# tensorflow/compression

Hardware: AMD Instinct MI355X
Metric: Mpixels/s encode+decode round-trip (bit-exact) (higher is better)
Workload: dtype int32

## Files before the change

compression_amd/csrc/range_pipe.h:

```cpp
#pragma once

#ifndef TFC_PIPE_TIMING
#define TFC_PIPE_TIMING 0
#endif

namespace tfc {

constexpr int kPipeTile = 256;
constexpr int kPipeEscMax = 32;
constexpr unsigned int kPipeBlock = 16;
constexpr unsigned int kPipeNoCall = 0x0001FFFFu;
constexpr unsigned int kPipeAggregate = 1u << 30;
constexpr unsigned int kPipePrefix = 2u << 30;
constexpr unsigned int kPipeRowsMask = (1u << 30) - 1u;

struct PipeEncArgs {
  const uint16_t* fast16;
  const int2* rows_fast;
  int ntab;
  int tab_entries;
  unsigned int* calls;
  unsigned int* status;
  unsigned int* done;
  unsigned int* fallback;
// ... 591 lines not shown
    const unsigned int dslot = b % L::kDigSlots;
    dstage = area + L::kDig + dslot * L::kDigSlot + L::kDigStride * lane;
    ds_off = area_off + L::kDig + dslot * L::kDigSlot + L::kDigStride * lane;
    n = 0u;
    block(wa);
    if (lane == 0u) sync[L::kConsumed] = b + 1u;
    if (!last) {
      seq = ((seq_early & ~(L::kLast | L::kBail)) == b + 2u || (seq_early & L::kBail)) ? seq_early : wait_words(b + 1u);
      if (seq & L::kBail) { bail = true; break; }
      read_words(wa, (b + 1u) % L::kSlots, 0u);
    }
    block(wb);
    reinterpret_cast<uint2*>(area + L::kRec)[dslot * 64u + lane] = make_uint2(wpos, n);
    overflow |= (n != 0u && wpos + ((n + 15u) & ~15u) > pa.cap) ? 1u : 0u;
    wpos += n;
    asm volatile("s_waitcnt lgkmcnt(0)" ::: "memory");
    if (lane == 0u) sync[L::kDigPub] = b + 1u;
    if (__any(too_long)) {
      bail = true;
      if (lane == 0u) atomicOr(&pa.fallback[job], 1u);
      break;
    }
    if (last) break;
  }
  asm volatile("s_waitcnt lgkmcnt(0)" ::: "memory");
  if (lane == 0u) sync[L::kExit] = 1u;
  if (gi == 0u && lane == 0u) {
    g_pipe_clock[0] = clock64() - clk0;
    g_pipe_clock[1] = wall_clock64() - wall0;
    g_pipe_clock[4] = waited_words;
    g_pipe_clock[6] = waited_digits;
#if TFC_PIPE_TIMING
    g_enc_clock[0] = t_blocks; g_enc_clock[1] = n_blocks; g_enc_clock[2] = n_redone; g_enc_clock[3] = t_redo;
#endif
  }
  if (bail) return;
  if (live) {
    pa.stage_state[static_cast<size_t>(gi) * 64 + lane] = make_uint4(base, s1, (hd & 0xFFFFu) | (had << 31), rn);
    pa.stage_out[static_cast<size_t>(gi) * 64 + lane] = make_uint2(wpos, overflow);
  }
}

__global__ void __launch_bounds__(64) enc_chain_direct_kernel(const PipeChainJobs jobs, const PipeEncArgs pa) {
  constexpr unsigned int kRows = PipeEncChainLds::kRows;
  constexpr unsigned int kDigits = 2 * kRows;
  constexpr int kStride = lane_stride(kDigits + 8);
  __shared__ __attribute__((aligned(16))) unsigned char stage[64 * kStride];
  const unsigned int gi = blockIdx.x;
  const unsigned int job = gi / static_cast<unsigned int>(pa.groups_per_job);
  const unsigned int gidx = gi % static_cast<unsigned int>(pa.groups_per_job);
  if (__hip_atomic_load(&pa.fallback[job], __ATOMIC_RELAXED, __HIP_MEMORY_SCOPE_AGENT) != 0u) return;
  const PipeChainJob& J = jobs.job[job];
  const unsigned int lane = threadIdx.x;
  const int64_t s = static_cast<int64_t>(gidx) * 64 + lane;
  const bool live = s < jobs.streams;

  uint4 st = live ? J.state[s] : make_uint4(0u, 0xFFFFFFFFu, 0u, 0u);
  unsigned int base = st.x, s1 = st.y, hd = st.z & 0xFFFFu, had = st.z >> 31, rn = st.w;
  lanes_pin(base, s1, hd, rn);

  const unsigned int ds_off = static_cast<unsigned int>(reinterpret_cast<size_t>(
                                  (__attribute__((address_space(3))) unsigned char*)stage)) + kStride * lane;
  unsigned char* const dstage = stage + kStride * lane;
  unsigned char* const out = J.chunk + (live ? s : 0) * static_cast<int64_t>(pa.cap);
  unsigned int wpos = 0u, n = 0u, overflow = 0u;

  auto put = [&](unsigned int d, bool on) {
    *reinterpret_cast<unsigned short*>(dstage + n) = __builtin_bswap16(static_cast<unsigned short>(d));
    n += on ? 2u : 0u;
  };
  auto flush = [&]() {
#pragma unroll
    for (unsigned int c = 0; c < kDigits / 16u; ++c) {
      if (16u * c < n) {
        uint2 v[2];
        v[0] = reinterpret_cast<const uint2*>(dstage)[2 * c];
        v[1] = reinterpret_cast<const uint2*>(dstage)[2 * c + 1];
        if (wpos + 16u * c + 16u <= pa.cap) lanes_gstore16(out + wpos + 16u * c, v[0], v[1]);
        else overflow = 1u;
      }
    }
    wpos += n;
    n = 0u;
  };
  auto put_run = [&](unsigned int fill, unsigned int bytes) {
    flush();
    for (unsigned int k = 0; k < bytes; k += 2u) {
      const unsigned short be = static_cast<unsigned short>(fill);
      if (wpos + 2u <= pa.cap) lanes_gstore_elem(reinterpret_cast<unsigned short*>(out + wpos), be);
      else overflow = 1u;
      wpos += 2u;
    }
  };
  auto call = [&](unsigned int lo, unsigned int hi, bool act) __attribute__((always_inline)) {
    const unsigned int a = scale16(s1, lo);
    const unsigned int b = scale16(s1, hi) - 1u;
    const unsigned int bs = base + a;
    const unsigned int t1 = b - a;
    const bool carry = act && bs < a;
    const bool ren = act && (t1 >> 16) == 0u;
    const unsigned int e = bs >> 16;
    const bool solid = ren && e != 0xFFFFu;
    const bool ffff = ren && e == 0xFFFFu;
    const bool held = had != 0u;
    const unsigned int X = (hd + (carry ? 1u : 0u)) & 0xFFFFu;
    const bool emit = held && (solid || (carry && (!ffff || rn != 0u)));
    put(X, emit);
    const unsigned int run_out = !held ? 0u : solid ? rn : (carry && rn != 0u) ? (ffff ? rn - 1u : rn) : 0u;
    if (__any(run_out != 0u)) {
      if (run_out != 0u) put_run(carry ? 0u : 0xFFFFu, 2u * run_out);
    }
    if (solid) {
      hd = e; had = 1u; rn = 0u;
    } else if (ffff) {
      if (!held) { hd = 0xFFFFu; had = 1u; rn = 0u; }
      else if (!carry) { rn += 1u; }
      else if (rn == 0u) { hd = X; rn = 1u; }
      else { hd = 0u; rn = 1u; }
    } else if (carry && held) {
      had = 0u; rn = 0u;
    }
    base = act ? (ren ? bs << 16 : bs) : base;
    s1 = act ? (ren ? (t1 << 16) | 0xFFFFu : t1) : s1;
  };

  const unsigned int nt = static_cast<unsigned int>(pa.nt);
  const unsigned int* const status = pa.status + static_cast<size_t>(gi) * nt * 64 + lane;
  const unsigned int* const done = pa.done + static_cast<size_t>(gi) * nt;
  unsigned int avail = 0u;
  unsigned int tn = 0u;
  bool bail = false;
  auto ensure = [&](unsigned int need) {
    while (tn < nt && __any(live && avail < need)) {
      const unsigned int* const flag = done + tn;
      long long t0 = 0;
      bool timing = false;
      while (__hip_atomic_load(flag, __ATOMIC_RELAXED, __HIP_MEMORY_SCOPE_AGENT) == 0u) {
        const long long now = static_cast<long long>(wall_clock64());
        if (!timing) { t0 = now; timing = true; }
        else if (now - t0 > pa.poll_ticks) { bail = true; return; }
        __builtin_amdgcn_s_sleep(8);
      }
      __builtin_amdgcn_fence(__ATOMIC_ACQUIRE, "agent");
      avail = __hip_atomic_load(status + static_cast<size_t>(tn) * 64, __ATOMIC_RELAXED, __HIP_MEMORY_SCOPE_AGENT) & kPipeRowsMask;
      ++tn;
      if (__hip_atomic_load(&pa.fallback[job], __ATOMIC_RELAXED, __HIP_MEMORY_SCOPE_AGENT) != 0u) { bail = true; return; }
    }
  };

  const unsigned char* const mine = reinterpret_cast<const unsigned char*>(pa.calls + static_cast<size_t>(gi) * 64 * pa.rows) + 128u * lane;
  unsigned int w[kRows] = {}, wn[kRows] = {};
  auto load_rows = [&](unsigned int b) {
    const unsigned char* p = mine + static_cast<size_t>(b) * (64u * kRows * 4u);
#pragma unroll
    for (unsigned int c = 0; c < kRows / 4u; ++c) {
      const uint4 v = lanes_gload16(p + 16u * c);
      wn[4 * c] = v.x; wn[4 * c + 1] = v.y; wn[4 * c + 2] = v.z; wn[4 * c + 3] = v.w;
    }
  };
  auto block = [&](unsigned int w0, unsigned int w1, unsigned int w2, unsigned int w3, unsigned int w4, unsigned int w5,
                   unsigned int w6, unsigned int w7, unsigned int w8, unsigned int w9, unsigned int w10, unsigned int w11,
                   unsigned int w12, unsigned int w13, unsigned int w14, unsigned int w15) __attribute__((always_inline)) {
    const unsigned int base0 = base, s10 = s1, hd0 = hd, had0 = had;
    unsigned int flag = rn, na = ds_off + n;
    asm volatile(
        "s_mov_b64 s[56:57], exec\n\t"
        "v_mov_b32 v101, 0\n\tv_mov_b32 v103, 0\n\t"
        TFC_PENC_STEP(W0) TFC_PENC_STEP(W1) TFC_PENC_STEP(W2) TFC_PENC_STEP(W3)
        TFC_PENC_STEP(W4) TFC_PENC_STEP(W5) TFC_PENC_STEP(W6) TFC_PENC_STEP(W7)
        TFC_PENC_STEP(W8) TFC_PENC_STEP(W9) TFC_PENC_STEP(W10) TFC_PENC_STEP(W11)
        TFC_PENC_STEP(W12) TFC_PENC_STEP(W13) TFC_PENC_STEP(W14) TFC_PENC_STEP(W15)
        "s_mov_b64 exec, s[56:57]\n\t"
        "s_waitcnt lgkmcnt(0)\n\t"
        : [BASE] "+v"(base), [S] "+v"(s1), [H] "+v"(hd), [HAD] "+v"(had), [NA] "+v"(na), [FLAG] "+v"(flag)
        : [NOCALL] "s"(kPipeNoCall), [K64K] "s"(0x10000u), [KFFFF] "s"(0xFFFFu), [PERM] "s"(0x0c0c0001u),
          [W0] "v"(w0), [W1] "v"(w1), [W2] "v"(w2), [W3] "v"(w3), [W4] "v"(w4), [W5] "v"(w5),
          [W6] "v"(w6), [W7] "v"(w7), [W8] "v"(w8), [W9] "v"(w9), [W10] "v"(w10), [W11] "v"(w11),
          [W12] "v"(w12), [W13] "v"(w13), [W14] "v"(w14), [W15] "v"(w15)
        : "vcc", "memory", "s52", "s53", "s56", "s57", "v100", "v101", "v102", "v103", "v104", "v105", "v106", "v107",
          "v108", "v109", "v110", "v111", "v112", "v113", "v114", "v115", "v117", "v118", "v119");
    if (__builtin_expect(!__any(flag != 0u), 1)) {
      n = na - ds_off;
    } else {
      base = base0; s1 = s10; hd = hd0; had = had0;
      const unsigned int ww[kPipeBlock] = {w0, w1, w2, w3, w4, w5, w6, w7, w8, w9, w10, w11, w12, w13, w14, w15};
#pragma nounroll
      for (unsigned int k = 0; k < kPipeBlock; ++k) {
        unsigned int word = ww[0];
#pragma unroll
        for (unsigned int q = 1; q < kPipeBlock; ++q) word = k == q ? ww[q] : word;
        const unsigned int hi = word >> 16;
        call(word & 0xFFFFu, hi == 0u ? 65536u : hi, word != kPipeNoCall);
      }
    }
  };

  ensure(kRows);
  if (!bail) load_rows(0u);
#pragma unroll
  for (unsigned int k = 0; k < kRows; ++k) asm volatile("" : "+v"(wn[k]));
  for (unsigned int b = 0; !bail && (tn < nt || __any(b * kRows < avail)); ++b) {
#pragma unroll
    for (unsigned int k = 0; k < kRows; ++k) w[k] = wn[k];
    ensure((b + 2u) * kRows);
    if (bail) break;
    load_rows(b + 1u);
    flush();
    if (__any(avail < (b + 1u) * kRows)) {
#pragma unroll
      for (unsigned int k = 0; k < kRows; ++k) w[k] = b * kRows + k < avail ? w[k] : kPipeNoCall;
    }
    block(w[0], w[1], w[2], w[3], w[4], w[5], w[6], w[7], w[8], w[9], w[10], w[11], w[12], w[13], w[14], w[15]);
    block(w[16], w[17], w[18], w[19], w[20], w[21], w[22], w[23], w[24], w[25], w[26], w[27], w[28], w[29], w[30], w[31]);
  }
  flush();
  if (bail) {
    if (lane == 0) atomicOr(&pa.fallback[job], 1u);
    return;
  }
  if (live) {
    pa.stage_state[static_cast<size_t>(gi) * 64 + lane] = make_uint4(base, s1, (hd & 0xFFFFu) | (had << 31), rn);
    pa.stage_out[static_cast<size_t>(gi) * 64 + lane] = make_uint2(wpos, overflow);
  }
}


__global__ void enc_gate_kernel(const unsigned int* started, unsigned int want, long long ticks) {
  const long long t0 = static_cast<long long>(wall_clock64());
  while (__hip_atomic_load(started, __ATOMIC_RELAXED, __HIP_MEMORY_SCOPE_AGENT) < want &&
         static_cast<long long>(wall_clock64()) - t0 < ticks)
    __builtin_amdgcn_s_sleep(8);
}

__global__ void __launch_bounds__(64) enc_commit_kernel(const PipeChainJobs jobs, const PipeEncArgs pa) {
  const unsigned int gi = blockIdx.x;
  const unsigned int job = gi / static_cast<unsigned int>(pa.groups_per_job);
  const unsigned int gidx = gi % static_cast<unsigned int>(pa.groups_per_job);
  if (pa.fallback[job] != 0u) return;
  const int64_t s = static_cast<int64_t>(gidx) * 64 + threadIdx.x;
  if (s >= jobs.streams) return;
  const PipeChainJob& J = jobs.job[job];
  J.state[s] = pa.stage_state[static_cast<size_t>(gi) * 64 + threadIdx.x];
  const uint2 o = pa.stage_out[static_cast<size_t>(gi) * 64 + threadIdx.x];
  J.chunk_len[s] = o.y ? 0u : o.x;
  if (o.y) atomicOr(J.overflow_flag, 1u);
}


constexpr unsigned int kPipeSkipRow = 0xFFFFu;
__device__ inline unsigned int pipe_raw_entry(unsigned int sym_or_bit, int M) { return (M != 0 ? 0x8000u : 0u) | sym_or_bit; }
__device__ inline int pipe_mode_step(int M, unsigned int bit) {
  if (M < 0) return bit ? -M : (M == -31 ? 32 : M - 1);
  return M - 1;
}

struct PipeDecArgs {
  unsigned short* raw;
  unsigned int* posrec;
  unsigned int* kend;
  uint4* state_out;
  const unsigned short* rowaddr;
  unsigned int* fallback;
  unsigned int* progress;
  unsigned int* tile_done;
  unsigned int* started;
  int rows;
  int groups_per_job;
  int groups;
  int concurrent;
  long long poll_ticks;
};
constexpr unsigned int kPipeFinal = 0x80000000u;
#ifndef TFC_PIPE_RELEASE
#define TFC_PIPE_RELEASE 64
#endif
constexpr unsigned int kPipeRelease = TFC_PIPE_RELEASE;
struct PipeDecJob { const uint8_t* blob; const long long* off; const uint4* state; };
struct PipeDecJobs {
  int64_t streams, elems;
  int blocks_per_job, n;
  PipeDecJob job[64];
};

struct PipeRowJobs {
  int64_t per_job;
  int ntab, n;
  struct { const int32_t* index; unsigned long long* first_error; } job[64];
};
__global__ void __launch_bounds__(256) dec_rows_kernel(const PipeRowJobs jobs, unsigned short* rowaddr) {
  const int k = blockIdx.y;
  const int32_t* index = jobs.job[k].index;
  unsigned short* out = rowaddr + static_cast<size_t>(k) * jobs.per_job;
  for (int64_t i = static_cast<int64_t>(blockIdx.x) * 1024 + threadIdx.x, e = min(jobs.per_job, (static_cast<int64_t>(blockIdx.x) + 1) * 1024);
       i < e; i += 256) {
    int t = tfc_gload(index + i);
    if (t < 0 || t >= jobs.ntab) {
      atomicMin(jobs.job[k].first_error, static_cast<unsigned long long>(i));
      t = 0;
    }
    out[i] = static_cast<unsigned short>(16 * t);
  }
}

struct PipeDecLds {
  static constexpr int kWords = 2 * kPipeBlock * 2 / 8 + 2;
  static constexpr int kStride = lane_stride(8 * kWords);
  static constexpr int kCodes = 0;
  static constexpr int kRows = kCodes + 64 * kStride;
  static constexpr int kBytes = kRows + 64 * kStride;
  static constexpr int kStage = kPipeBlock * 128;
};

#ifndef TFC_PDEC_ABL
#define TFC_PDEC_ABL 0
#endif
#if TFC_PDEC_ABL & 1
#define TFC_PDEC_STORE(KOFF)
#define TFC_PDEC_WAIT2 "s_waitcnt lgkmcnt(1)\n\t"
#else
#define TFC_PDEC_STORE(KOFF) "ds_write_b16 %[STG], v117 offset:" #KOFF "\n\t"
#define TFC_PDEC_WAIT2 "s_waitcnt lgkmcnt(2)\n\t"
#endif
#ifndef TFC_PDEC_PAD
#define TFC_PDEC_PAD 0
#endif
#define TFC_PDEC_PAD2 "v_mov_b32 v139, v139\n\tv_mov_b32 v139, v139\n\t"
#if TFC_PDEC_PAD == 1
#define TFC_PDEC_PAD_A TFC_PDEC_PAD2
#elif TFC_PDEC_PAD == 5
#define TFC_PDEC_PAD_A "s_waitcnt lgkmcnt(15)\n\ts_waitcnt lgkmcnt(15)\n\t"
#else
#define TFC_PDEC_PAD_A
#endif
#if TFC_PDEC_PAD == 2
#define TFC_PDEC_PAD_B TFC_PDEC_PAD2
#else
#define TFC_PDEC_PAD_B
#endif
#if TFC_PDEC_PAD == 3
#define TFC_PDEC_PAD_C TFC_PDEC_PAD2
#else
#define TFC_PDEC_PAD_C
#endif
#if TFC_PDEC_PAD == 4
#define TFC_PDEC_PAD_D TFC_PDEC_PAD2
#else
#define TFC_PDEC_PAD_D
#endif
#define TFC_PDEC_STEP(KOFF, MI, MO, AHEAD, NEXT, PWSTEP)                                    \
  "v_cvt_f32_u32 v111, %[S]\n\t"                                                          \
  "v_add_f32 v111, 1.0, v111\n\t"                                                         \
  "v_rcp_f32 v111, v111\n\t"                                                              \
  TFC_PDEC_PAD_A                                                                          \
  "v_cvt_f32_u32 v110, %[D]\n\t"                                                          \
  "v_fma_f32 v110, -v110, %[SCALE], -%[HSCALE]\n\t"                                       \
  "v_fma_f32 v110, v110, v111, -1.0\n\t"                                                  \
  "v_cvt_i32_f32 v110, v110\n\t"                                                          \
  "v_ashrrev_i32 v111, 6, v110\n\t"                                                       \
  "s_waitcnt lgkmcnt(0)\n\t"                                                              \
  "v_mad_i32_i24 v112, v111, -8, v106\n\t"                                                \
  "ds_read_b64 v[114:115], v112\n\t"                                                      \
  "v_mad_i32_i24 v113, v111, -2, v107\n\t"                                                \
  "ds_read_u16 v116, v113\n\t"                                                            \
  AHEAD                                                                                   \
  "v_cndmask_b32_e64 v133, 0, 2, s[56:57]\n\t"                                            \
  "v_add_u32 %[CP], %[CP], v133\n\t"                                                      \
  "ds_read_u16 v109, %[CP]\n\t"                                                           \
  "v_ashrrev_i32 v137, 31, " MI "\n\t"                                                    \
  "v_cmp_le_u32_sdwa vcc, v110, v105 src0_sel:WORD_0 src1_sel:WORD_1\n\t"                 \
  "v_cndmask_b32 v137, v136, v137, vcc\n\t"                                               \
  "v_xor_b32 " MO ", v135, v137\n\t"                                                      \
  "v_cmpx_le_u32 vcc, v130, v131\n\t"                                                     \
  TFC_PDEC_PAD_B                                                                          \
  "s_waitcnt lgkmcnt(1)\n\t"                                                              \
  "v_lshlrev_b64 v[118:119], v110, v[114:115]\n\t"                                        \
  "v_bcnt_u32_b32 v116, v118, v116\n\t"                                                   \
  "v_bcnt_u32_b32 v117, v119, v116\n\t"                                                   \
  "v_lshl_add_u32 v112, v117, 1, v104\n\t"                                                \
  "ds_read_u16 v122, v112 offset:2\n\t"                                                   \
  "ds_read_u16 v124, v112 offset:4\n\t"                                                   \
  TFC_PDEC_PAD_C                                                                          \
  TFC_PDEC_STORE(KOFF)                                                                    \
  "v_subrev_co_u32 v135, vcc, 1, " MO "\n\t"                                              \
  "v_cndmask_b32_e64 v136, 0, -1, vcc\n\t"                                                \
  "v_add_u32 v140, " #PWSTEP ", %[PW]\n\t"                                                \
  "v_cndmask_b32 %[PW], %[PW], v140, vcc\n\t"                                             \
  "v_cndmask_b32 v142, %[BINROW], " NEXT ", vcc\n\t"                                      \
  "ds_read_b128 v[104:107], v142\n\t"                                                     \
  TFC_PDEC_WAIT2                                                                          \
  TFC_PDEC_PAD_D                                                                          \
  "v_mad_u64_u32 v[126:127], s[52:53], v122, %[S], v[122:123]\n\t"                        \
  "v_mad_u64_u32 v[128:129], s[52:53], v124, %[S], v[124:125]\n\t"                        \
  "v_alignbit_b32 v126, v127, v126, 16\n\t"                                               \
  "v_alignbit_b32 v128, v129, v128, 16\n\t"                                               \
  "v_add_u32 v128, -1, v128\n\t"                                                          \
  "v_min_u32 v128, v128, %[S]\n\t"                                                        \
  "v_sub_u32 v131, v128, v126\n\t"                                                        \
  "v_cmp_gt_u32_e64 s[56:57], %[K64K], v131\n\t"                                          \
  "v_lshl_or_b32 v132, v131, 16, %[KFFFF]\n\t"                                            \
  "v_cndmask_b32_e64 %[S], v131, v132, s[56:57]\n\t"                                      \
  "v_sub_u32 v130, %[D], v126\n\t"                                                        \
  "v_perm_b32 v132, v130, v109, %[PERM]\n\t"                                              \
  "v_cndmask_b32_e64 %[D], v130, v132, s[56:57]\n\t"
#define TFC_PDEC_STEP_H(KOFF, MI, MO, AHEAD, NEXT, PWSTEP)                                  \
  "v_cvt_f32_u32 v111, %[S]\n\t"                                                          \
  "v_add_f32 v111, 1.0, v111\n\t"                                                         \
  "v_rcp_f32 v111, v111\n\t"                                                              \
  "v_cvt_f32_u32 v110, %[D]\n\t"                                                          \
  "v_fma_f32 v110, -v110, %[SCALE], -%[HSCALE]\n\t"                                       \
  "v_fma_f32 v110, v110, v111, -1.0\n\t"                                                  \
  "v_cvt_i32_f32 v110, v110\n\t"                                                          \
  "v_ashrrev_i32 v143, 1, v110\n\t"                                                       \
  "v_ashrrev_i32 v111, 6, v143\n\t"                                                       \
  "s_waitcnt lgkmcnt(0)\n\t"                                                              \
  "v_mad_i32_i24 v112, v111, -8, v106\n\t"                                                \
  "ds_read_b64 v[114:115], v112\n\t"                                                      \
  "v_mad_i32_i24 v113, v111, -2, v107\n\t"                                                \
  "ds_read_u16 v116, v113\n\t"                                                            \
  AHEAD                                                                                   \
  "v_cndmask_b32_e64 v133, 0, 2, s[56:57]\n\t"                                            \
  "v_add_u32 %[CP], %[CP], v133\n\t"                                                      \
  "ds_read_u16 v109, %[CP]\n\t"                                                           \
  "v_ashrrev_i32 v137, 31, " MI "\n\t"                                                    \
  "v_cmp_le_u32_sdwa vcc, v110, v105 src0_sel:WORD_0 src1_sel:WORD_1\n\t"                 \
  "v_cndmask_b32 v137, v136, v137, vcc\n\t"                                               \
  "v_xor_b32 " MO ", v135, v137\n\t"                                                      \
  "v_cmpx_le_u32 vcc, v130, v131\n\t"                                                     \
  "v_mad_i32_i24 v141, v110, %[NSH], %[NSH]\n\t"                                          \
  "s_waitcnt lgkmcnt(1)\n\t"                                                              \
  "v_lshlrev_b64 v[118:119], v143, v[114:115]\n\t"                                        \
  "v_bcnt_u32_b32 v116, v118, v116\n\t"                                                   \
  "v_bcnt_u32_b32 v117, v119, v116\n\t"                                                   \
  "v_lshl_add_u32 v112, v117, 2, v104\n\t"                                                \
  "ds_read2_b32 v[144:145], v112 offset1:1\n\t"                                           \
  "v_subrev_co_u32 v135, vcc, 1, " MO "\n\t"                                              \
  "v_cndmask_b32_e64 v136, 0, -1, vcc\n\t"                                                \
  "v_add_u32 v140, " #PWSTEP ", %[PW]\n\t"                                                \
  "v_cndmask_b32 %[PW], %[PW], v140, vcc\n\t"                                             \
  "v_cndmask_b32 v142, %[BINROW], " NEXT ", vcc\n\t"                                      \
  "ds_read_b128 v[104:107], v142\n\t"                                                     \
  "s_waitcnt lgkmcnt(1)\n\t"                                                              \
  "v_cmp_ge_u32_sdwa vcc, v141, v144 src0_sel:DWORD src1_sel:WORD_1\n\t"                  \
  "v_cndmask_b32_sdwa v122, v144, v144, vcc dst_sel:DWORD dst_unused:UNUSED_PAD src0_sel:WORD_0 src1_sel:WORD_1\n\t" \
  "v_cndmask_b32_sdwa v124, v144, v145, vcc dst_sel:DWORD dst_unused:UNUSED_PAD src0_sel:WORD_1 src1_sel:WORD_0\n\t" \
  "v_addc_co_u32_e64 v117, s[58:59], v117, v117, vcc\n\t"                                 \
  "v_cmp_ge_u32_sdwa vcc, v141, v145 src0_sel:DWORD src1_sel:WORD_0\n\t"                  \
  "v_cndmask_b32_sdwa v122, v122, v145, vcc dst_sel:DWORD dst_unused:UNUSED_PAD src0_sel:DWORD src1_sel:WORD_0\n\t" \
  "v_cndmask_b32_sdwa v124, v124, v145, vcc dst_sel:DWORD dst_unused:UNUSED_PAD src0_sel:DWORD src1_sel:WORD_1\n\t" \
  "v_addc_co_u32_e64 v117, s[58:59], v117, v123, vcc\n\t"                                 \
  TFC_PDEC_STORE(KOFF)                                                                    \
  "v_mad_u64_u32 v[126:127], s[52:53], v122, %[S], v[122:123]\n\t"                        \
  "v_mad_u64_u32 v[128:129], s[52:53], v124, %[S], v[124:125]\n\t"                        \
  "v_alignbit_b32 v126, v127, v126, 16\n\t"                                               \
  "v_alignbit_b32 v128, v129, v128, 16\n\t"                                               \
  "v_add_u32 v128, -1, v128\n\t"                                                          \
  "v_min_u32 v128, v128, %[S]\n\t"                                                        \
  "v_sub_u32 v131, v128, v126\n\t"                                                        \
  "v_cmp_gt_u32_e64 s[56:57], %[K64K], v131\n\t"                                          \
  "v_lshl_or_b32 v132, v131, 16, %[KFFFF]\n\t"                                            \
  "v_cndmask_b32_e64 %[S], v131, v132, s[56:57]\n\t"                                      \
  "v_sub_u32 v130, %[D], v126\n\t"                                                        \
  "v_perm_b32 v132, v130, v109, %[PERM]\n\t"                                              \
  "v_cndmask_b32_e64 %[D], v130, v132, s[56:57]\n\t"
#define TFC_PDEC_STEP_CH(KOFF, MI, MO) TFC_PDEC_STEP(KOFF, MI, MO, "", "v140", 16)
#define TFC_PDEC_STEP_IX(KOFF, MI, MO) TFC_PDEC_STEP(KOFF, MI, MO, "ds_read_u16 v108, %[PW] offset:2\n\t", "v108", 2)
#define TFC_PDEC_STEP_PCH(KOFF, MI, MO) TFC_PDEC_STEP_H(KOFF, MI, MO, "", "v140", 16)
#define TFC_PDEC_STEP_PIX(KOFF, MI, MO) TFC_PDEC_STEP_H(KOFF, MI, MO, "ds_read_u16 v108, %[PW] offset:2\n\t", "v108", 2)
#define TFC_PDEC_STEP2(STEP, K0, K1) STEP(K0, "%[M]", "v138") STEP(K1, "v138", "%[M]")
#define TFC_PDEC_BLOCK_HEAD                                                               \
  "v_mov_b32 v104, %[R0]\n\tv_mov_b32 v105, %[R1]\n\tv_mov_b32 v106, %[R2]\n\tv_mov_b32 v107, %[R3]\n\t" \
  "v_mov_b32 v123, 0\n\tv_mov_b32 v125, 0\n\t"                                           \
  "v_mov_b32 v130, 0\n\tv_mov_b32 v131, 0\n\ts_mov_b64 s[56:57], 0\n\t"                   \
  "v_subrev_co_u32 v135, vcc, 1, %[M]\n\tv_cndmask_b32_e64 v136, 0, -1, vcc\n\t"           \
  "s_mov_b64 s[54:55], exec\n\tv_mov_b32 %[FLAG], 1\n\t"
#define TFC_PDEC_BLOCK_TAIL                                                               \
  "v_cndmask_b32_e64 v133, 0, 2, s[56:57]\n\t"                                            \
  "v_add_u32 %[CP], %[CP], v133\n\t"                                                      \
  "s_waitcnt lgkmcnt(0)\n\t"                                                              \
  "v_cmpx_le_u32 vcc, v130, v131\n\tv_mov_b32 %[FLAG], 0\n\ts_mov_b64 exec, s[54:55]\n\t"   \
  "v_mov_b32 %[R0], v104\n\tv_mov_b32 %[R1], v105\n\tv_mov_b32 %[R2], v106\n\tv_mov_b32 %[R3], v107\n\t"
#define TFC_PDEC_ONE(STEP) TFC_PDEC_BLOCK_HEAD STEP(0, "%[M]", "v138") "v_mov_b32 %[M], v138\n\t" TFC_PDEC_BLOCK_TAIL
#define TFC_PDEC_BLOCK(STEP)                                                              \
  TFC_PDEC_BLOCK_HEAD                                                                     \
  TFC_PDEC_STEP2(STEP, 0, 128) TFC_PDEC_STEP2(STEP, 256, 384) TFC_PDEC_STEP2(STEP, 512, 640)            \
  TFC_PDEC_STEP2(STEP, 768, 896) TFC_PDEC_STEP2(STEP, 1024, 1152) TFC_PDEC_STEP2(STEP, 1280, 1408)      \
  TFC_PDEC_STEP2(STEP, 1536, 1664) TFC_PDEC_STEP2(STEP, 1792, 1920)                       \
  TFC_PDEC_BLOCK_TAIL

template <bool INDEXED, bool PAIRS>
__global__ void __launch_bounds__(512) dec_chain_kernel(const PipeDecJobs jobs, const LaneArgs la, const PipeDecArgs pa) {
  extern __shared__ unsigned char lanes_lds[];
  lanes_load_image(lanes_lds, la);
  using L = PipeDecLds;
  if constexpr (!PAIRS) {
    const unsigned int entries = static_cast<unsigned int>(la.ntab) + kLaneDirRepeat + 1u;
    const unsigned int nw = max(1u, (1u << la.precision) >> 6) + 1u;
    for (unsigned int i = threadIdx.x; i < entries; i += blockDim.x) {
      if (i >= static_cast<unsigned int>(la.ntab) && i + 1u != entries) continue;
      const LaneRow* e = reinterpret_cast<const LaneRow*>(lanes_lds) + i;
      *reinterpret_cast<unsigned long long*>(lanes_lds + e->bits) &= ~1ull;
      *reinterpret_cast<unsigned short*>(lanes_lds + e->cum) = 0;
    }
    __syncthreads();
    {
      const LaneRow* e = reinterpret_cast<const LaneRow*>(lanes_lds) + (entries - 1u);
      for (unsigned int w = threadIdx.x; w < nw; w += blockDim.x)
        *reinterpret_cast<unsigned short*>(lanes_lds + e->cum + 2u * w) += 0x8000u;
    }
    __syncthreads();
    for (unsigned int i = threadIdx.x; i < entries; i += blockDim.x) {
      LaneRow* e = reinterpret_cast<LaneRow*>(lanes_lds) + i;
      const unsigned int info = e->info, limit = info & 0x7FFFu, esc = info >> 31;
      unsigned int esclo = 0xFFFFu;
      if (i + 1u == entries) esclo = 1u << (la.precision - 1);
      else if (esc) esclo = lds_u16(lanes_lds, e->cdf + 2u * limit + 2u) >> (16 - la.precision);
      e->info = limit | (esc << 15) | ((0xFFFFu - esclo) << 16);
      e->bits -= 8u;
      e->cum -= 2u;
      if (i + 1u == entries) e->cdf -= 0x10000u;
    }
    __syncthreads();
  }

  const unsigned long long clk0 = clock64(), wall0 = wall_clock64();
  if (threadIdx.x == 0u) __hip_atomic_fetch_add(pa.started, 1u, __ATOMIC_RELAXED, __HIP_MEMORY_SCOPE_AGENT);
  const unsigned int job = blockIdx.x / static_cast<unsigned int>(jobs.blocks_per_job);
  const unsigned int wv = (blockIdx.x % static_cast<unsigned int>(jobs.blocks_per_job)) * (blockDim.x >> 6) + (threadIdx.x >> 6);
  if (wv >= static_cast<unsigned int>(pa.groups_per_job)) return;
  const unsigned int gi = job * static_cast<unsigned int>(pa.groups_per_job) + wv;
  const PipeDecJob& J = jobs.job[job];
  const unsigned int lane = threadIdx.x & 63u;
  const int64_t s = static_cast<int64_t>(wv) * 64 + lane;
  const bool live = s < jobs.streams;
  const unsigned int elems = live ? static_cast<unsigned int>(jobs.elems) : 0u;

  const uint4 st = live ? J.state[s] : make_uint4(0u, 0xFFFFFFFFu, 0u, 2u);
  unsigned int D = st.z - st.x;
  unsigned int s1 = st.y;
  const long long o0 = live ? J.off[s] : 0;
  unsigned int len = live ? static_cast<unsigned int>(J.off[s + 1] - o0) : 0u;
  unsigned int pos_start = 2u * st.w;
  lanes_pin(D, s1, len, pos_start);

  const unsigned int lds0 = static_cast<unsigned int>(reinterpret_cast<size_t>(
      (__attribute__((address_space(3))) unsigned char*)lanes_lds));
  const unsigned int wave_off = static_cast<unsigned int>(la.lds_image) + (threadIdx.x >> 6) * static_cast<unsigned int>(la.lds_wave);
  LaneWindow<L::kWords> cw;
  const unsigned int cw_off = wave_off + L::kCodes + L::kStride * lane;
  cw.lds = lanes_lds + cw_off;
  cw.g = J.blob + o0;
  cw.len = len;
  cw.request(pos_start);
  cw.base = pos_start;
  unsigned int cp = cw_off;
  LaneWindow<L::kWords> iw;
  const unsigned int iw_off = wave_off + L::kRows + L::kStride * lane;
  if (INDEXED) {
    iw.lds = lanes_lds + iw_off;
    iw.g = reinterpret_cast<const unsigned char*>(pa.rowaddr + (static_cast<size_t>(job) * jobs.streams + (live ? s : 0)) * jobs.elems);
    iw.len = elems * 2u;
    iw.request(0u);
    iw.base = 0u;
  }

  const unsigned int stg_off = wave_off + (INDEXED ? L::kBytes : L::kRows);
  const unsigned int stg = stg_off + 2u * lane;
  bool staged = false;
  unsigned int staged_k = 0u;

  const float scale = static_cast<float>(1u << la.precision);
  float hscale = scale;
  asm volatile("" : "+v"(hscale));
  const unsigned int cp_max = (1u << la.precision) - 1u;
  const unsigned int pair_sh = 16u - static_cast<unsigned int>(la.precision);
  const unsigned int pair_nsh = 0u - (1u << pair_sh);
  const unsigned int dir_end = 16u * static_cast<unsigned int>(la.ntab);
  const unsigned int bin_addr = dir_end + 16u * kLaneDirRepeat;
  uint4 bin = *reinterpret_cast<const uint4*>(lanes_lds + bin_addr);
  asm volatile("" : "+v"(bin.x), "+v"(bin.y), "+v"(bin.z), "+v"(bin.w));
  unsigned int bin_addr_v = bin_addr;
  asm volatile("" : "+v"(bin_addr_v));

  unsigned int pos = 0u;
  int M = 0;
  unsigned int pw = INDEXED ? iw_off : 0u;
  uint4 R = make_uint4(0u, 0u, 0u, 0u);
  bool row_loaded = false;

  unsigned short* const raw = pa.raw + static_cast<size_t>(gi) * pa.rows * 64;
  unsigned int* const posrec = pa.posrec + static_cast<size_t>(gi) * (pa.rows / kPipeBlock + 1) * 64 + lane;
  unsigned int k = 0u;
  auto flush = [&]() {
    if (!staged) return;
#if TFC_PDEC_ABL & 4
    staged = false;
    return;
#endif
    unsigned char* dst = reinterpret_cast<unsigned char*>(raw + static_cast<size_t>(staged_k) * 64) + 16u * lane;
#pragma unroll
    for (unsigned int j = 0; j < L::kStage / 1024u; ++j) {
      const uint4 v = *reinterpret_cast<const uint4*>(lanes_lds + stg_off + 1024u * j + 16u * lane);
      lanes_gstore16(dst + 1024u * j, make_uint2(v.x, v.y), make_uint2(v.z, v.w));
    }
    staged = false;
  };

  auto load_row = [&]() {
    const unsigned int a = INDEXED ? static_cast<unsigned int>(*reinterpret_cast<const unsigned short*>(lanes_lds + pw)) : pw;
    R = *reinterpret_cast<const uint4*>(lanes_lds + a);
  };

  auto gstep = [&](bool act, unsigned int row, bool to_stage = false) {
    unsigned int entry = 0u;
    if (act) {
      const unsigned int dig = __builtin_bswap16(*reinterpret_cast<const unsigned short*>(lanes_lds + cp));
      if (M == 0) {
        const float fq = (static_cast<float>(D) + 0.5f) * __builtin_amdgcn_rcpf(static_cast<float>(s1)) * scale;
        const unsigned int q = min(static_cast<unsigned int>(fq), cp_max);
        if constexpr (PAIRS) {
          const unsigned int j = q >> 1, w = j >> 6;
          const unsigned long long word = *reinterpret_cast<const unsigned long long*>(lanes_lds + R.z + 8u + 8u * w);
          const unsigned int cum = *reinterpret_cast<const unsigned short*>(lanes_lds + R.w + 2u + 2u * w);
          const unsigned long long below = ~0ull >> (63u - (j & 63u));
          const unsigned int i = cum + static_cast<unsigned int>(__popcll(word & below));
          const unsigned int Q = q << pair_sh;
          unsigned int u = 2u * i;
          u += Q >= lds_u16(lanes_lds, R.x + 2u * u + 2u) ? 1u : 0u;
          u += (u & 1u) != 0u && Q >= lds_u16(lanes_lds, R.x + 4u * i + 4u) ? 1u : 0u;
          unsigned int lo = lds_u16(lanes_lds, R.x + 2u * u), hi = lds_u16(lanes_lds, R.x + 2u * u + 2u);
          unsigned int A = scale16(s1, lo);
          unsigned int b = scale16(s1, hi) - 1u;
          b = hi == 0u ? s1 : b;
          for (int fix = 0; fix < 4; ++fix) {
            if (D - A > b - A) {
              if (D < A) u = u > 0u ? u - 1u : 0u;
              else if (hi != 0u) u = u + 1u;
              lo = lds_u16(lanes_lds, R.x + 2u * u);
              hi = lds_u16(lanes_lds, R.x + 2u * u + 2u);
              A = scale16(s1, lo);
              b = scale16(s1, hi) - 1u;
              b = hi == 0u ? s1 : b;
            }
          }
          D -= A;
          s1 = b - A;
          const bool ren = (s1 >> 16) == 0u;
          D = ren ? (D << 16) | dig : D;
          s1 = ren ? (s1 << 16) | 0xFFFFu : s1;
          cp += ren ? 2u : 0u;
          entry = u;
          M = ((R.y >> 15) & 1u) != 0u && lo == ((0xFFFFu - (R.y >> 16)) << pair_sh) ? -1 : 0;
        } else {
        const unsigned int w = q >> 6;
        const unsigned long long word = *reinterpret_cast<const unsigned long long*>(lanes_lds + R.z + 8u + 8u * w);
        const unsigned int cum = *reinterpret_cast<const unsigned short*>(lanes_lds + R.w + 2u + 2u * w);
        const unsigned long long below = ~0ull >> (63u - (q & 63u));
        unsigned int sym = cum + static_cast<unsigned int>(__popcll(word & below));
        unsigned int lo = lds_u16(lanes_lds, R.x + 2u * sym + 2u);
        unsigned int hi = lds_u16(lanes_lds, R.x + 2u * sym + 4u);
        unsigned int A = scale16(s1, lo);
        unsigned int b = scale16(s1, hi) - 1u;
        b = hi == 0u ? s1 : b;
        const unsigned int nsym = (R.y & 0x7FFFu) + ((R.y >> 15) & 1u);
        for (int fix = 0; fix < 4; ++fix) {
          if (D - A > b - A) {
            if (D < A) sym = sym > 0u ? sym - 1u : 0u;
            else sym = sym + 1u < nsym ? sym + 1u : nsym - 1u;
            lo = lds_u16(lanes_lds, R.x + 2u * sym + 2u);
            hi = lds_u16(lanes_lds, R.x + 2u * sym + 4u);
            A = scale16(s1, lo);
            b = scale16(s1, hi) - 1u;
            b = hi == 0u ? s1 : b;
          }
        }
        D -= A;
        s1 = b - A;
        const bool ren = (s1 >> 16) == 0u;
        D = ren ? (D << 16) | dig : D;
        s1 = ren ? (s1 << 16) | 0xFFFFu : s1;
        cp += ren ? 2u : 0u;
        entry = pipe_raw_entry(sym, 0);
        M = ((R.y >> 15) & 1u) != 0u && sym == (R.y & 0x7FFFu) ? -1 : 0;
        }
      } else {
        const unsigned int half = scale16(s1, 32768u);
        const unsigned int bit = D >= half ? 1u : 0u;
        const unsigned int A = bit ? half : 0u;
        const unsigned int b = bit ? s1 : half - 1u;
        D -= A;
        s1 = b - A;
        const bool ren = (s1 >> 16) == 0u;
        D = ren ? (D << 16) | dig : D;
        s1 = ren ? (s1 << 16) | 0xFFFFu : s1;
        cp += ren ? 2u : 0u;
        entry = PAIRS ? 0x8001u + bit : pipe_raw_entry(bit, M);
        if (M < 0) {
          if (bit) M = -M;
          else M = M == -31 ? 32 : M - 1;
        } else {
          --M;
        }
      }
      if (M == 0) {
        ++pos;
        pw += INDEXED ? 2u : 16u;
        if (!INDEXED && pw == dir_end) pw = 0u;
        load_row();
      } else {
        R = bin;
      }
      if (to_stage) *reinterpret_cast<unsigned short*>(lanes_lds + stg + 128u * (row - k)) = static_cast<unsigned short>(entry);
      else raw[static_cast<size_t>(row) * 64 + lane] = static_cast<unsigned short>(entry);
    }
  };

#if TFC_PIPE_TIMING
  unsigned long long t_asm = 0ull, n_asm = 0ull, t_commit = 0ull, t_rest = 0ull;
#endif
  auto memory_phase = [&]() __attribute__((always_inline)) {
#if TFC_PIPE_TIMING
    const unsigned long long tm0 = clock64();
#endif
    const unsigned int cpos = cw.base + (cp - cw_off);
    cw.commit();
    cp = cw_off + (cpos - cw.base);
    if (INDEXED) {
      iw.commit();
      pw = iw_off + (2u * pos - iw.base);
    }
#if TFC_PIPE_TIMING
    asm volatile("s_waitcnt lgkmcnt(0)" ::: "memory");
    const unsigned long long tm1 = clock64();
    t_commit += tm1 - tm0;
#endif
    flush();
    if (k != 0u && (k / kPipeBlock) % kPipeRelease == 0u) {
      posrec[static_cast<size_t>(k / kPipeBlock) * 64] = pos + (M != 0 ? 1u : 0u);
      __builtin_amdgcn_fence(__ATOMIC_RELEASE, "agent");
      if (lane == 0u) __hip_atomic_store(&pa.progress[gi], k, __ATOMIC_RELAXED, __HIP_MEMORY_SCOPE_AGENT);
    }
    cw.request(cpos);
    if (INDEXED) iw.request(2u * pos);
    posrec[static_cast<size_t>(k / kPipeBlock) * 64] = pos + (M != 0 ? 1u : 0u);
#if TFC_PIPE_TIMING
    t_rest += clock64() - tm1;
#endif
  };
  auto fast_block = [&](unsigned int& flag) __attribute__((always_inline)) {
#define TFC_PDEC_OPERANDS                                                                                              \
        : [D] "+v"(D), [S] "+v"(s1), [CP] "+v"(cp), [M] "+v"(M), [PW] "+v"(pw), [FLAG] "+v"(flag),                    \
          [R0] "+v"(R.x), [R1] "+v"(R.y), [R2] "+v"(R.z), [R3] "+v"(R.w)                                              \
        : [STG] "v"(stg), [BINROW] "v"(bin_addr_v), [SCALE] "s"(scale), [HSCALE] "v"(hscale),        \
          [K64K] "s"(0x10000u), [KFFFF] "s"(0xFFFFu), [PERM] "s"(0x05040001u), [NSH] "s"(pair_nsh) \
        : "vcc", "memory", "s52", "s53", "s54", "s55", "s56", "s57", "s58", "s59", "v104", "v105", "v106", "v107", "v108", "v109", "v110", "v111", "v112", "v113", \
          "v114", "v115", "v116", "v117", "v118", "v119", "v122", "v123", "v124", "v125", "v126", "v127", "v128",      \
          "v129", "v130", "v131", "v132", "v133", "v134", "v135", "v136", "v137", "v138", "v139", "v140", "v141", "v142", "v143", "v144", "v145"
#if TFC_PIPE_TIMING
    const unsigned long long ta = clock64();
#endif
    if constexpr (INDEXED && PAIRS) asm volatile(TFC_PDEC_BLOCK(TFC_PDEC_STEP_PIX) TFC_PDEC_OPERANDS);
    else if constexpr (PAIRS) asm volatile(TFC_PDEC_BLOCK(TFC_PDEC_STEP_PCH) TFC_PDEC_OPERANDS);
    else if constexpr (INDEXED) asm volatile(TFC_PDEC_BLOCK(TFC_PDEC_STEP_IX) TFC_PDEC_OPERANDS);
    else asm volatile(TFC_PDEC_BLOCK(TFC_PDEC_STEP_CH) TFC_PDEC_OPERANDS);
#if TFC_PIPE_TIMING
    t_asm += clock64() - ta;
    ++n_asm;
#endif
  };
  auto fast_step = [&](unsigned int& flag, unsigned int slot) __attribute__((always_inline)) {
    const unsigned int stg_row = stg + 128u * slot;
    {
      const unsigned int stg = stg_row;
      if constexpr (INDEXED && PAIRS) asm volatile(TFC_PDEC_ONE(TFC_PDEC_STEP_PIX) TFC_PDEC_OPERANDS);
      else if constexpr (PAIRS) asm volatile(TFC_PDEC_ONE(TFC_PDEC_STEP_PCH) TFC_PDEC_OPERANDS);
      else if constexpr (INDEXED) asm volatile(TFC_PDEC_ONE(TFC_PDEC_STEP_IX) TFC_PDEC_OPERANDS);
      else asm volatile(TFC_PDEC_ONE(TFC_PDEC_STEP_CH) TFC_PDEC_OPERANDS);
    }
#undef TFC_PDEC_OPERANDS
  };
  bool gave_up = false;
  while (__any(pos < elems)) {
    if (lds0 == 0u && row_loaded && (INDEXED || static_cast<unsigned int>(la.ntab) >= kPipeBlock)) {
      while (__all(!live || (pos + kPipeBlock <= elems && M > -16)) && k + kPipeBlock <= static_cast<unsigned int>(pa.rows)) {
        memory_phase();
        const unsigned int D0 = D, s10 = s1, cp0 = cp, pw0 = pw;
        const int M0 = M;
        const uint4 R0 = R;
        unsigned int flag = 0u;
        fast_block(flag);
        if (__builtin_expect(__any(live && flag != 0u), 0)) {
          D = D0; s1 = s10; cp = cp0; pw = pw0; M = M0; R = R0;
#pragma nounroll
          for (unsigned int i = 0; i < kPipeBlock; ++i) {
            const unsigned int D1 = D, s11 = s1, cp1 = cp, pw1 = pw;
            const int M1 = M;
            const uint4 R1 = R;
            unsigned int f1 = 0u;
            if (live) fast_step(f1, i);
            if (__any(live && f1 != 0u)) {
              D = D1; s1 = s11; cp = cp1; pw = pw1; M = M1; R = R1;
              gstep(live, k + i, true);
            } else {
              pos += (pw - pw1) / (INDEXED ? 2u : 16u);
              if (!INDEXED) pw -= pw >= dir_end ? dir_end : 0u;
            }
          }
          staged = true;
          staged_k = k;
          k += kPipeBlock;
          continue;
        }
        pos += (pw - pw0) / (INDEXED ? 2u : 16u);
        if (!INDEXED) pw -= pw >= dir_end ? dir_end : 0u;
        staged = true;
        staged_k = k;
        k += kPipeBlock;
      }
      if (!__any(pos < elems)) break;
    }
    if (k + kPipeBlock > static_cast<unsigned int>(pa.rows)) {
      gave_up = true;
      break;
    }
    memory_phase();
    if (!row_loaded) {
      if (M == 0) load_row(); else R = bin;
      row_loaded = true;
    }
    const bool whole = pos + kPipeBlock <= elems;
    const bool blocks = __any(whole);
    if (blocks && __any(!whole && pos < elems && M != 0)) {
      if (pos < elems) {
#pragma unroll
        for (unsigned int i = 0; i < kPipeBlock; ++i) raw[static_cast<size_t>(k + i) * 64 + lane] = static_cast<unsigned short>(kPipeSkipRow);
      }
#pragma nounroll
      for (unsigned int i = 0; i < kPipeBlock; ++i) gstep(!whole && pos < elems && M != 0, k + i);
      k += kPipeBlock;
      continue;
    }
    const bool busy = blocks ? whole : pos < elems;
    const bool sitting = blocks && !whole && pos < elems;
    if (__builtin_expect(lds0 == 0u && blocks && !__any(busy && M <= -16), 1)) {
      if (__any(sitting)) {
        if (sitting) {
#pragma unroll
          for (unsigned int i = 0; i < kPipeBlock; ++i) *reinterpret_cast<unsigned short*>(lanes_lds + stg + 128u * i) = static_cast<unsigned short>(kPipeSkipRow);
        }
      }
      const unsigned int D0 = D, s10 = s1, cp0 = cp, pw0 = pw;
      const int M0 = M;
      const uint4 R0 = R;
      unsigned int flag = 0u;
      if (busy) {
        fast_block(flag);
      }
      if (__builtin_expect(!__any(flag != 0u), 1)) {
        if (busy) {
          pos += (pw - pw0) / (INDEXED ? 2u : 16u);
        }
        if (!INDEXED)
          while (__any(busy && pw >= dir_end)) pw -= pw >= dir_end ? dir_end : 0u;
        staged = true;
        staged_k = k;
        k += kPipeBlock;
        continue;
      }
      D = D0; s1 = s10; cp = cp0; pw = pw0; M = M0; R = R0;
    }
    if (sitting) {
#pragma unroll
      for (unsigned int i = 0; i < kPipeBlock; ++i) raw[static_cast<size_t>(k + i) * 64 + lane] = static_cast<unsigned short>(kPipeSkipRow);
    }
#pragma nounroll
    for (unsigned int i = 0; i < kPipeBlock; ++i) gstep(busy && pos < elems, k + i);
    k += kPipeBlock;
  }
  flush();
  posrec[static_cast<size_t>(k / kPipeBlock) * 64] = pos;
  if (gave_up) {
    if (lane == 0) {
      atomicOr(&pa.fallback[job], 1u);
      __hip_atomic_store(&pa.progress[gi], kPipeFinal, __ATOMIC_RELEASE, __HIP_MEMORY_SCOPE_AGENT);
    }
    return;
  }
  if (lane == 0) pa.kend[gi] = k;
  __builtin_amdgcn_fence(__ATOMIC_RELEASE, "agent");
  if (lane == 0) __hip_atomic_store(&pa.progress[gi], k | kPipeFinal, __ATOMIC_RELAXED, __HIP_MEMORY_SCOPE_AGENT);
  if (gi == 0 && lane == 0) {
    g_pipe_clock[2] = clock64() - clk0;
    g_pipe_clock[3] = wall_clock64() - wall0;
#if TFC_PIPE_TIMING
    g_pipe_clock[5] = t_asm | (t_commit << 32);
    g_pipe_clock[7] = n_asm | (static_cast<unsigned long long>(k) << 16) | (t_rest << 32);
#endif
  }
  if (live) {
    const unsigned int cpos = cw.base + (cp - cw_off);
    const unsigned char* srcp = J.blob + o0;
    unsigned int window = 0u;
    for (int i = -4; i < 0; ++i) {
      const long long q = static_cast<long long>(cpos) + i;
      window = (window << 8) | ((q >= 0 && q < static_cast<long long>(len)) ? srcp[q] : 0u);
    }
    pa.state_out[static_cast<size_t>(gi) * 64 + lane] = make_uint4(window - D, s1, window, cpos >> 1);
  }
}

constexpr int kParseRows = 128;
constexpr unsigned int kParseMargin = 96;

constexpr int kParseEscTables = 2048;

struct PipePairMap { const int* adjust; };
template <bool INDEXED, bool PAIRS, typename Dst>
__global__ void __launch_bounds__(256) dec_parse_kernel(const DecLaneJobs<Dst> jobs, const PipeDecArgs pa, const DecRow* dir, int ntab,
                                                        const PipePairMap pm) {
  constexpr int kPitch = 66;
  __shared__ unsigned short buf[kParseRows * kPitch];
  __shared__ unsigned int escsym[kParseEscTables];
  __shared__ unsigned int incomplete;
  const unsigned int tiles = static_cast<unsigned int>(pa.rows) / kParseRows + 1u;
  const unsigned int gi = blockIdx.x % static_cast<unsigned int>(pa.groups), kt = blockIdx.x / static_cast<unsigned int>(pa.groups);
  const unsigned int job = gi / static_cast<unsigned int>(pa.groups_per_job);
  const unsigned int wv = gi % static_cast<unsigned int>(pa.groups_per_job);
  const DecLaneJob<Dst>& J = jobs.job[job];
  const unsigned int tid = threadIdx.x, lane = tid & 63u;
  const unsigned int k0 = kt * kParseRows;
  unsigned int* const tile_done = pa.tile_done + static_cast<size_t>(gi) * tiles + kt;
  unsigned int kend;
  bool final = true;
  if (pa.concurrent) {
    const unsigned int need = k0 + kParseRows + kParseMargin;
    unsigned int* const abandon = pa.started + 1;
    unsigned int v = 0u;
    if (tid == 0u) {
      unsigned int seen = ~0u, go = 1u;
      long long t0 = 0;
      if (__hip_atomic_load(abandon, __ATOMIC_RELAXED, __HIP_MEMORY_SCOPE_AGENT) != 0u) go = 0u;
      while (go) {
        v = __hip_atomic_load(&pa.progress[gi], __ATOMIC_RELAXED, __HIP_MEMORY_SCOPE_AGENT);
        if ((v & kPipeFinal) || v >= need) break;
        const long long now = static_cast<long long>(wall_clock64());
        if (v != seen) { seen = v; t0 = now; }
        else if (now - t0 > pa.poll_ticks) {
          __hip_atomic_store(abandon, 1u, __ATOMIC_RELAXED, __HIP_MEMORY_SCOPE_AGENT);
          go = 0u;
          break;
        }
        __builtin_amdgcn_s_sleep(32);
      }
      incomplete = go ? v : 0xFFFFFFFFu;
    }
    __syncthreads();
    v = incomplete;
    __syncthreads();
    if (v == 0xFFFFFFFFu) return;
    __builtin_amdgcn_fence(__ATOMIC_ACQUIRE, "agent");
    if (__hip_atomic_load(&pa.fallback[job], __ATOMIC_RELAXED, __HIP_MEMORY_SCOPE_AGENT) != 0u) return;
    final = (v & kPipeFinal) != 0u;
    kend = v & ~kPipeFinal;
    if (tid == 0u) incomplete = 0u;
  } else {
    if (pa.fallback[job] != 0u) return;
    if (kt == 0u && tid < 64u) {
      const int64_t s = static_cast<int64_t>(wv) * 64 + tid;
      if (s < jobs.streams) J.state[s] = pa.state_out[static_cast<size_t>(gi) * 64 + tid];
    }
    if (*tile_done != 0u) return;
    kend = pa.kend[gi];
  }
  if (k0 >= kend) return;
  const unsigned short* const raw = pa.raw + static_cast<size_t>(gi) * pa.rows * 64;
  const unsigned int nrows = min(static_cast<unsigned int>(kParseRows), kend - k0);
  for (unsigned int r = tid >> 6; r < nrows; r += 4u) buf[r * kPitch + lane] = raw[static_cast<size_t>(k0 + r) * 64 + lane];
  const bool esc_lds = ntab <= kParseEscTables;
  if (esc_lds)
    for (int i = tid; i < ntab; i += 256) {
      escsym[i] = (static_cast<unsigned int>(dir[i].w) & 0xFFFFu) | (PAIRS ? static_cast<unsigned int>(pm.adjust[i] + 2) << 16 : 0u);
    }
  __syncthreads();
  const unsigned int bitshift = PAIRS ? 1u : 0u;
  const unsigned int* const posrec = pa.posrec + static_cast<size_t>(gi) * (pa.rows / kPipeBlock + 1) * 64;
  const Dst dst = J.dst;
  const unsigned long long lt = (1ull << lane) - 1ull;
  const unsigned int untab = static_cast<unsigned int>(ntab);
  auto walk = [&](auto in_lds) __attribute__((always_inline)) {
  constexpr bool esc_in_lds = decltype(in_lds)::value;
  for (unsigned int l = tid >> 6; l < 64u; l += 4u) {
    const int64_t s = static_cast<int64_t>(wv) * 64 + l;
    if (s >= jobs.streams) continue;
    unsigned int p = posrec[static_cast<size_t>(k0 / kPipeBlock) * 64 + l];
    const unsigned int p1 = posrec[static_cast<size_t>((k0 + nrows) / kPipeBlock) * 64 + l];
    const int64_t base = s * jobs.elems;
    unsigned int pmod = p % untab;
    for (unsigned int c = 0; c < nrows; c += 64u) {
      const unsigned int i = c + lane;
      const unsigned int e = i < nrows ? buf[i * kPitch + l] : kPipeSkipRow;
      const bool start = (e & 0x8000u) == 0u;
      const unsigned long long mask = __ballot(start);
      const unsigned int before = static_cast<unsigned int>(__popcll(mask & lt));
      const unsigned int ord = p + before;
      const unsigned int total = static_cast<unsigned int>(__popcll(mask));
      if (start && ord < p1) {
        const int64_t at = base + ord;
        int t;
        if (INDEXED) {
          t = tfc_gload(J.index + at);
          t = (t < 0 || t >= ntab) ? 0 : t;
        } else {
          unsigned int m = pmod + before;
          if (untab >= 64u) m -= m >= untab ? untab : 0u;
          else m %= untab;
          t = static_cast<int>(m);
        }
        int v = static_cast<int>(e);
        const unsigned int ew = esc_in_lds ? escsym[t] : 0u;
        if constexpr (PAIRS) v += esc_in_lds ? static_cast<int>(ew >> 16) - 2 : pm.adjust[t];
        const int es = esc_in_lds ? static_cast<int>(static_cast<short>(ew & 0xFFFFu)) : dir[t].w;
        if (v == es) {
          unsigned int val = 0u;
          bool neg = false, closed = false;
          int m = -1;
          for (unsigned int q = k0 + i + 1u; q < kend; ++q) {
            const unsigned int x = q - k0 < nrows ? buf[(q - k0) * kPitch + l]
                                                  : *reinterpret_cast<const TFC_AS1 unsigned short*>((const TFC_AS1 void*)(raw + static_cast<size_t>(q) * 64 + l));
            const unsigned int bit = (x >> bitshift) & 1u;
            if (x == kPipeSkipRow) continue;
            if (m < 0) {
              if (bit) val = 1u << (-m - 1);
              else if (m == -31) val = 1u << 31;
            } else if (m > 1) {
              val |= bit << (m - 2);
            } else {
              neg = bit != 0u;
              closed = true;
              break;
            }
            m = pipe_mode_step(m, bit);
          }
          if (!closed && !final) incomplete = 1u;
          v = neg ? -static_cast<int>(val) : static_cast<int>(val) + es - 1;
        }
        dst.store(at, t, v);
      }
      p += total;
      pmod = (pmod + total) % untab;
    }
  }
  };
  if (esc_lds) walk(std::true_type{}); else walk(std::false_type{});
  if (pa.concurrent) {
    __syncthreads();
    if (tid == 0u && incomplete == 0u) *tile_done = 1u;
  }
}

}
```

Measured before the change: 62260.

## Replace decoder code window with a mirrored LDS ring buffer refilled incrementally

The per-lane compressed-byte window in the pipelined decoder becomes an 80-byte LDS ring with a 32-byte mirror, replacing the sliding LaneWindow. Each memory phase now loads and commits only the 0-2 16-byte chunks actually consumed, where before the whole window was reloaded and rewritten. This is meant to cut global load and LDS write traffic per block. In exchange it adds ring-offset bookkeeping, an extra mirror store, and a data-dependent branch. It also changes the LDS layout stride for the code region.

```diff
diff --git a/compression_amd/csrc/range_pipe.h b/compression_amd/csrc/range_pipe.h
--- a/compression_amd/csrc/range_pipe.h
+++ b/compression_amd/csrc/range_pipe.h
@@ -917,11 +917,79 @@
   }
 }
 
+struct PipeCodeRing {
+  static constexpr unsigned int kRing = 80, kMirror = 32, kBytes = kRing + kMirror;
+  unsigned char* lds;
+  const unsigned char* g;
+  unsigned int len;
+  unsigned int rbase;
+  unsigned int next;
+  unsigned int slot;
+  unsigned int pslot;
+  unsigned int npend;
+  uint4 pend[kRing / 16];
+
+  __device__ __noinline__ uint4 tail_chunk(unsigned int q0) const {
+    unsigned int w[4] = {0u, 0u, 0u, 0u};
+#pragma nounroll
+    for (unsigned int k = 0; k < 16u; ++k)
+      if (q0 + k < len) w[k >> 2] |= static_cast<unsigned int>(lanes_gload8(g + q0 + k)) << (8u * (k & 3u));
+    return make_uint4(w[0], w[1], w[2], w[3]);
+  }
+  __device__ uint4 chunk(unsigned int q0) const { return q0 + 16u <= len ? lanes_gload16(g + q0) : tail_chunk(q0); }
+  __device__ void put(unsigned int off, const uint4& v) {
+    *reinterpret_cast<uint4*>(lds + off) = v;
+    if (off < kMirror) *reinterpret_cast<uint4*>(lds + off + kRing) = v;
+  }
+  __device__ void request_all(unsigned int pos) {
+#pragma unroll
+    for (unsigned int c = 0; c < kRing / 16u; ++c) pend[c] = chunk(pos + 16u * c);
+    rbase = pos;
+    next = pos + kRing;
+    slot = 0u;
+    pslot = 0u;
+    npend = kRing / 16u;
+  }
+  template <bool FIRST>
+  __device__ void commit() {
+    if constexpr (FIRST) {
+#pragma unroll
+      for (unsigned int c = 0; c < kRing / 16u; ++c) put(16u * c, pend[c]);
+    } else {
+      if (npend >= 1u) put(pslot, pend[0]);
+      if (npend >= 2u) put(pslot + 16u == kRing ? 0u : pslot + 16u, pend[1]);
+    }
+    npend = 0u;
+  }
+  __device__ void request(unsigned int cpos) {
+    const unsigned int gap = next - cpos;
+    const unsigned int n = gap >= 64u ? 0u : gap >= 48u ? 1u : 2u;
+    pslot = slot;
+    if (__builtin_expect(__any(next + 32u > len), 0)) {
+      pend[0] = chunk(next);
+      pend[1] = chunk(next + 16u);
+    } else {
+      pend[0] = lanes_gload16(g + next);
+      pend[1] = lanes_gload16(g + next + 16u);
+    }
+    next += 16u * n;
+    slot += 16u * n;
+    slot -= slot >= kRing ? kRing : 0u;
+    npend = n;
+  }
+  __device__ unsigned int pos(unsigned int off) const { return rbase + off; }
+  __device__ unsigned int off(unsigned int cpos) {
+    if (cpos - rbase >= kRing) rbase += kRing;
+    return cpos - rbase;
+  }
+};
+
 struct PipeDecLds {
   static constexpr int kWords = 2 * kPipeBlock * 2 / 8 + 2;
   static constexpr int kStride = lane_stride(8 * kWords);
+  static constexpr int kCodeStride = PipeCodeRing::kBytes;
   static constexpr int kCodes = 0;
-  static constexpr int kRows = kCodes + 64 * kStride;
+  static constexpr int kRows = kCodes + 64 * kCodeStride;
   static constexpr int kBytes = kRows + 64 * kStride;
   static constexpr int kStage = kPipeBlock * 128;
 };
@@ -1160,13 +1228,13 @@
   const unsigned int lds0 = static_cast<unsigned int>(reinterpret_cast<size_t>(
       (__attribute__((address_space(3))) unsigned char*)lanes_lds));
   const unsigned int wave_off = static_cast<unsigned int>(la.lds_image) + (threadIdx.x >> 6) * static_cast<unsigned int>(la.lds_wave);
-  LaneWindow<L::kWords> cw;
-  const unsigned int cw_off = wave_off + L::kCodes + L::kStride * lane;
+  PipeCodeRing cw;
+  const unsigned int cw_off = wave_off + L::kCodes + L::kCodeStride * lane;
   cw.lds = lanes_lds + cw_off;
   cw.g = J.blob + o0;
   cw.len = len;
-  cw.request(pos_start);
-  cw.base = pos_start;
+  cw.request_all(pos_start);
+  bool cw_first = true;
   unsigned int cp = cw_off;
   LaneWindow<L::kWords> iw;
   const unsigned int iw_off = wave_off + L::kRows + L::kStride * lane;
@@ -1336,9 +1404,11 @@
 #if TFC_PIPE_TIMING
     const unsigned long long tm0 = clock64();
 #endif
-    const unsigned int cpos = cw.base + (cp - cw_off);
-    cw.commit();
-    cp = cw_off + (cpos - cw.base);
+    const unsigned int cpos = cw.pos(cp - cw_off);
+    if (cw_first) cw.commit<true>();
+    else cw.commit<false>();
+    cw_first = false;
+    cp = cw_off + cw.off(cpos);
     if (INDEXED) {
       iw.commit();
       pw = iw_off + (2u * pos - iw.base);
@@ -1512,7 +1582,7 @@
 #endif
   }
   if (live) {
-    const unsigned int cpos = cw.base + (cp - cw_off);
+    const unsigned int cpos = cw.pos(cp - cw_off);
     const unsigned char* srcp = J.blob + o0;
     unsigned int window = 0u;
     for (int i = -4; i < 0; ++i) {
```

New measurement: 62160, median of 2. No clear change (-0.2%).
